# pygda-team/pygda

Hardware: AMD Instinct MI355X
Metric: edges_aggregated_per_sec (higher is better)
Workload: dtype f32

## Files before the change

include/gda_hip.h:

```cpp
#ifndef GDA_HIP_H
#define GDA_HIP_H

#include <stddef.h>
#include <stdint.h>

#ifdef __cplusplus
extern "C" {
#endif

#define GDA_OK 0
#define GDA_E_NULL (-1)
#define GDA_E_SIZE (-2)
#define GDA_E_WORKSPACE (-3)
#define GDA_E_UNSUPPORTED (-4)
#define GDA_E_ALIAS (-5)
#define GDA_E_RCCL (-100)

typedef void* gda_stream_t;

int gda_abi_version(void);
const char* gda_status_string(int status);

size_t gda_graph_workspace_bytes(int64_t E, int64_t N);
int gda_build_csr_norm(const int64_t* src, const int64_t* dst, const float* w,
// ... 430 lines not shown
                             const int32_t* idx_s, const int32_t* idx_t, const float* alpha, int64_t n_i,
                             int a, float dropout_p, uint64_t seed, const int64_t* step, uint32_t site,
                             float gp_weight, float* loss, const gda_adam_tensor* params ,
                             float lr, float beta1, float beta2, float eps, float weight_decay,
                             void* workspace, size_t workspace_bytes, gda_stream_t stream);

#define GDA_GEMM_NT 0
#define GDA_GEMM_NN 1
#define GDA_GEMM_TN 2
size_t gda_gemm_workspace_bytes(int mode, int64_t M, int64_t N, int64_t K);
int gda_gemm_f32(int mode, int64_t M, int64_t N, int64_t K, const float* A, int64_t lda,
                 const float* B, int64_t ldb, float* C, int64_t ldc,
                 void* workspace, size_t workspace_bytes, gda_stream_t stream);
int gda_gemm_ex_f32(int mode, int64_t M, int64_t N, int64_t K, const float* A, int64_t lda,
                    const float* B, int64_t ldb, float* C, int64_t ldc, const float* bias, float* colsum,
                    void* workspace, size_t workspace_bytes, gda_stream_t stream);
size_t gda_gemm_tall_workspace_bytes(int mode, int64_t M, int64_t N, int64_t K);
size_t gda_gemm_skinny_workspace_bytes(int mode, int64_t M, int64_t N, int64_t K);
int gda_gemm_skinny_f32(int mode, int64_t M, int64_t N, int64_t K, const float* A, int64_t lda,
                        const float* B, int64_t ldb, float* C, int64_t ldc, const float* bias, float* colsum,
                        void* workspace, size_t workspace_bytes, gda_stream_t stream);
int gda_gemm_nn_mask_f32(int64_t M, int64_t N, int64_t K, const float* A, int64_t lda, const float* B, int64_t ldb,
                         float* C, int64_t ldc, const float* y, int64_t ldm, float p, gda_stream_t stream);
int gda_gemm_tall_fwd_ex_f32(int64_t M, int64_t N, int64_t K, const float* A, int64_t lda, const int64_t* arow,
                             const float* B, int64_t ldb, float* C, int64_t ldc, const float* bias,
                             int act_mode, float p, uint64_t seed, const int64_t* step_dev, uint32_t site0,
                             uint32_t site1, gda_stream_t stream);
int gda_gemm_tall_wgrad_gather_f32(int64_t N, int64_t Krows, const float* A, int64_t lda, const float* X, int64_t ldx,
                                   const int64_t* xrow, float* C, int64_t ldc, float* colsum,
                                   void* workspace, size_t workspace_bytes, gda_stream_t stream);
int gda_gemm_tall_f32(int mode, int64_t M, int64_t N, int64_t K, const float* A, int64_t lda,
                      const float* B, int64_t ldb, float* C, int64_t ldc, const float* bias, float* colsum,
                      void* workspace, size_t workspace_bytes, gda_stream_t stream);


size_t gda_softmax_nll_workspace_bytes(void);
int gda_softmax_entropy_fwd_f32(const float* logits, int64_t ld, int64_t N, int C, float clamp_min, float* loss,
                                void* workspace, size_t workspace_bytes, gda_stream_t stream);
int gda_softmax_entropy_bwd_f32(const float* logits, int64_t ld, int64_t N, int C, float clamp_min,
                                const float* grad_loss, float* grad_logits, int64_t ldg, gda_stream_t stream);
int gda_softmax_nll_fwd_f32(const float* logits, int64_t ld, const int64_t* labels, int64_t N, int C,
                            float* loss, void* workspace, size_t workspace_bytes, gda_stream_t stream);
int gda_softmax_nll_fwd_ex_f32(const float* logits, int64_t ld, const int64_t* labels, int64_t N, int C,
                               float* loss, double* stats, void* workspace, size_t workspace_bytes,
                               gda_stream_t stream);
int gda_softmax_nll_bwd_f32(const float* logits, int64_t ld, const int64_t* labels, int64_t N, int C,
// ... 148 lines not shown
```

pygda_amd/_lib.py:

```python
import ctypes
import os
from ctypes import c_char_p, c_float, c_int, c_int64, c_size_t, c_void_p

import torch

HERE = os.path.dirname(os.path.abspath(__file__))
LIB_PATH = os.path.join(HERE, "libgda_hip.so")

class _P(c_void_p):

    @classmethod
    def from_param(cls, obj):
        if isinstance(obj, torch.Tensor):
            return c_void_p(obj.data_ptr())
        if obj is None:
            return None
        if isinstance(obj, str):
            raise TypeError("a str is not a pointer argument")
        return c_void_p.from_param(obj)


_SIGNATURES = {
    "gda_abi_version": (c_int, []),
    "gda_status_string": (c_char_p, [c_int]),
# ... 89 lines not shown
                                   _P, _P, _P, c_float, _P, _P, _P, c_int64, _P, _P, _P, c_int64, _P,
                                   _P, c_size_t, _P]),
    "gda_mmd_fused_nseg": (c_int, [c_int, c_int64, c_int64, c_float, c_int]),
    "gda_mmd_fused_layout": (c_int, [c_int, c_int64, c_int64, _P, c_int]),
    "gda_mmd_fused_fwd_f32": (c_int, [_P, c_int64, _P, c_int64, c_int64, _P, _P, c_int, c_int64, c_float, c_int, c_float,
                                      c_float, _P, _P, _P, _P, _P, _P, c_int, _P, c_size_t, _P]),
    "gda_mmd_fused_bwd_f32": (c_int, [_P, c_int, c_int, c_int64, c_int64, _P, c_float, _P,
                                      _P, _P, c_int64, _P, _P, _P, c_int64, _P, _P]),
    "gda_mmd_fused_bwd_mask_f32": (c_int, [_P, c_int, c_int, c_int64, c_int64, _P, c_float, _P,
                                           _P, _P, c_int64, _P, _P, _P, c_int64, _P, _P, c_float, _P, c_float, _P]),
    "gda_copy_from_pinned": (c_int, [_P, _P, c_size_t, _P]),
    "gda_softmax_entropy_fwd_f32": (c_int, [_P, c_int64, c_int64, c_int, c_float, _P, _P, c_size_t, _P]),
    "gda_softmax_entropy_bwd_f32": (c_int, [_P, c_int64, c_int64, c_int, c_float, _P, _P, c_int64, _P]),
    "gda_mmd_chunked_plan": (c_int, [c_int, c_int64, c_int64, c_float, c_int, _P, c_int]),
    "gda_mmd_chunked_workspace_bytes": (c_size_t, [c_int, c_int64, c_int64]),
    "gda_mmd_chunked_fwd_f32": (c_int, [_P, c_int64, _P, c_int64, c_int64, _P, _P, c_int, c_int64, c_float, c_int, c_float,
                                        c_float, _P, _P, _P, c_int64, _P, _P, _P, c_int64, c_int, _P, c_size_t, _P]),
    "gda_mmd_fused_bwd_ld_f32": (c_int, [_P, c_int64, c_int, c_int, c_int64, c_int64, _P, c_float, _P,
                                         _P, _P, c_int64, _P, _P, _P, c_int64, _P, _P, c_float, _P, c_float, _P]),
    "gda_gemm_tall_fwd_ex_f32": (c_int, [c_int64, c_int64, c_int64, _P, c_int64, _P, _P, c_int64, _P, c_int64, _P, c_int,
                                         c_float, ctypes.c_uint64, _P, ctypes.c_uint32, ctypes.c_uint32, _P]),
    "gda_gemm_tall_wgrad_gather_f32": (c_int, [c_int64, c_int64, _P, c_int64, _P, c_int64, _P, _P, c_int64, _P, _P, c_size_t, _P]),
    "gda_gemm_nn_mask_f32": (c_int, [c_int64, c_int64, c_int64, _P, c_int64, _P, c_int64, _P, c_int64, _P, c_int64, c_float, _P]),
    "gda_grl_disc_workspace_bytes": (c_size_t, [c_int64, c_int64, c_int]),
    "gda_grl_mlp_ce_workspace_bytes": (c_size_t, [c_int64, c_int64]),
    "gda_lsgan_head_workspace_bytes": (c_size_t, [c_int64]),
    "gda_lsgan_head_fwd_f32": (c_int, [_P, c_int64, c_int64, c_int64, _P, _P, c_float, _P, _P, _P, c_size_t, _P]),
    "gda_lsgan_head_bwd_f32": (c_int, [_P, c_int64, c_int64, c_int64, _P, _P, c_float, _P, _P, c_int64, _P, _P,
                                       _P, c_size_t, _P]),
    "gda_grl_mlp_ce_fwd_f32": (c_int, [_P, c_int64, c_int64, _P, c_int64, c_int64, c_int64, c_int64, _P, _P, _P, _P,
                                       c_float, ctypes.c_uint64, _P, ctypes.c_uint32, _P, _P, c_size_t, _P]),
    "gda_grl_mlp_ce_bwd_f32": (c_int, [_P, c_int64, c_int64, _P, c_int64, c_int64, c_int64, c_int64, _P, _P, _P, _P,
                                       c_float, ctypes.c_uint64, _P, ctypes.c_uint32, _P, c_int, c_float, _P,
                                       _P, _P, _P, _P, _P, _P, _P, c_size_t, _P]),
    "gda_mlp_head_fwd_f32": (c_int, [c_int, _P, c_int64, c_int64, _P, c_int64, c_int64, c_int64, c_int64, _P, _P, _P, _P,
                                     c_float, ctypes.c_uint64, _P, ctypes.c_uint32, _P, _P, c_size_t, _P]),
    "gda_mlp_head_bwd_f32": (c_int, [c_int, _P, c_int64, c_int64, _P, c_int64, c_int64, c_int64, c_int64, _P, _P, _P, _P,
                                     c_float, ctypes.c_uint64, _P, ctypes.c_uint32, _P, c_int, c_float, _P,
                                     _P, _P, _P, _P, _P, _P, _P, c_size_t, _P]),
    "gda_grl_disc_ce_fwd_f32": (c_int, [_P, c_int64, c_int64, _P, c_int64, c_int64, c_int64, c_int,
                                        _P, _P, _P, _P, _P, _P, c_size_t, _P]),
    "gda_grl_disc_ce_bwd_f32": (c_int, [_P, c_int64, c_int64, _P, c_int64, c_int64, c_int64, c_int,
                                        _P, _P, _P, _P, c_float, _P, _P, _P, _P, _P, c_size_t, _P]),
    "gda_relu_dropout_fwd_f32": (c_int, [_P, _P, c_int64, c_float, ctypes.c_uint64, _P, ctypes.c_uint32, _P]),
    "gda_relu_dropout_bwd_f32": (c_int, [_P, _P, _P, c_int64, c_float, _P]),
    "gda_relu_dropout_tiled_fwd_f32": (c_int, [_P, c_int64, c_int64, _P, c_float, ctypes.c_uint64, _P, ctypes.c_uint32, _P]),
# ... 237 lines not shown
```

pygda_amd/csrc/gda_gemm.hip:

```cpp
#include "gda_common.h"
#include "gda_dropout.h"

#include <cstdlib>

namespace {

constexpr int TB = 256;
constexpr int TILE = 64;
constexpr int DK = 32;
constexpr int LDT = TILE + 4;
constexpr int PF = 4;

using f32x16 = __attribute__((ext_vector_type(16))) float;

__device__ __forceinline__ float4 ld4(const float* __restrict__ p, int64_t ld, int64_t r, int64_t c,
                                      int64_t rows, int64_t cols, bool vec) {
    float4 v = make_float4(0.f, 0.f, 0.f, 0.f);
    if (r >= rows) return v;
    const float* q = p + r * ld + c;
    if (vec && c + 3 < cols) return *reinterpret_cast<const float4*>(q);
    if (c + 0 < cols) v.x = q[0];
    if (c + 1 < cols) v.y = q[1];
    if (c + 2 < cols) v.z = q[2];
    if (c + 3 < cols) v.w = q[3];
// ... 508 lines not shown
        float c = 0.f;
#pragma unroll
        for (int q = 0; q < SK_N; ++q) if (q == n) { a = acc[q]; c = cs[q]; }
        *reinterpret_cast<float4*>(red + 4 * threadIdx.x) = a;
        __syncthreads();
        if (rl == 0) {
            float4 t = make_float4(0.f, 0.f, 0.f, 0.f);
            for (int r = 0; r < rlanes; ++r) {
                const float4 u = *reinterpret_cast<const float4*>(red + 4 * (r * pieces + p));
                t.x += u.x; t.y += u.y; t.z += u.z; t.w += u.w;
            }
            *reinterpret_cast<float4*>(out + (int64_t)n * K + 4 * p) = t;
        }
        if (CS) {
            __syncthreads();
            if (p == 0) red[rl] = c;
            __syncthreads();
            if (threadIdx.x == 0) {
                float t = 0.f;
                for (int r = 0; r < rlanes; ++r) t += red[r];
                CS[(int64_t)blockIdx.x * N + n] = t;
            }
        }
    }
}

bool vec_ok(const float* p, int64_t ld) { return ld % 4 == 0 && ((uintptr_t)p & 15) == 0; }

int slabs_for(int64_t K) {
    const int per = 128, cap = 256;
    int64_t s = gda_cdiv(K, per);
    if (s < 1) s = 1;
    if (s > cap) s = cap;
    return (int)s;
}

}

bool split_k(int mode, int64_t M, int64_t N, int64_t K) {
    return mode == GDA_GEMM_TN || (mode == GDA_GEMM_NN && K >= 1024 && M <= 512 && N <= 512);
}

extern "C" size_t gda_gemm_workspace_bytes(int mode, int64_t M, int64_t N, int64_t K) {
    if (M <= 0 || N <= 0 || K <= 0 || !split_k(mode, M, N, K)) return 0;
    const int s = slabs_for(K);
    return s > 1 ? (size_t)s * (size_t)M * (size_t)(N + 1) * sizeof(float) : 0;
// ... 197 lines not shown
        k_skinny_fwd<<<(unsigned)blocks, TB, 0, stream>>>(A, lda, B, ldb, bias, C, ldc, M, (int)N, (int)K);
    } else if (mode == GDA_GEMM_NN) {
        if (K > SK_N || !wide_ok(N) || bias || colsum || !al(B, ldb) || !al(C, ldc) || lda < K || ldb < N) return GDA_E_UNSUPPORTED;
        const int64_t rpb = TB / (N / 4);
        const int64_t blocks = min(gda_cdiv(M, rpb), (int64_t)256 * 16);
        k_skinny_dgrad<<<(unsigned)blocks, TB, 0, stream>>>(A, lda, B, ldb, C, ldc, M, (int)K, (int)N);
    } else if (mode == GDA_GEMM_TN) {
        if (M > SK_N || !wide_ok(N) || bias || !al(B, ldb) || lda < M || ldb < N) return GDA_E_UNSUPPORTED;
        const int64_t slabs = skinny_slabs(K);
        const int64_t rows = gda_cdiv(K, slabs);
        if (!workspace || workspace_bytes < gda_gemm_skinny_workspace_bytes(mode, M, N, K)) return GDA_E_WORKSPACE;
        float* part = (float*)workspace;
        float* cs_part = part + (size_t)slabs * M * N;
        k_skinny_wgrad<<<(unsigned)slabs, TB, 0, stream>>>(A, lda, B, ldb, part, colsum ? cs_part : nullptr, K, rows, (int)M, (int)N);
        GDA_LAUNCH_CHECK();
        GDA_UNLESS_SKIPPED("k_slab_sum") k_slab_sum<<<(unsigned)gda_cdiv(M * N + (colsum ? M : 0), SS_OUT), TB, 0, stream>>>(part, (int)slabs, M, N, C, ldc, cs_part, colsum);
    } else {
        return GDA_E_UNSUPPORTED;
    }
    GDA_LAUNCH_CHECK();
    return GDA_OK;
}

extern "C" int gda_gemm_nn_mask_f32(int64_t M, int64_t N, int64_t K, const float* A, int64_t lda, const float* B, int64_t ldb,
                                    float* C, int64_t ldc, const float* y, int64_t ldm, float p, gda_stream_t stream_) {
    if (M <= 0 || N <= 0 || K <= 0 || ldc < N || ldm < N || lda < K || ldb < N) return GDA_E_SIZE;
    if (!A || !B || !C || !y) return GDA_E_NULL;
    if (C == A || C == B || C == y) return GDA_E_ALIAS;
    if (!(p >= 0.f && p < 1.f)) return GDA_E_SIZE;
    if (ldc % 4 || ldm % 4 || ldb % 4 || (((uintptr_t)C | (uintptr_t)y | (uintptr_t)B) & 15)) return GDA_E_UNSUPPORTED;
    hipStream_t stream = (hipStream_t)stream_;
    const float mscale = 1.f / (1.f - p);
    if (K <= SK_N && (N == 32 || N == 64 || N == 128 || N == 256)) {
        const int64_t rpb = TB / (N / 4);
        const int64_t blocks = min(gda_cdiv(M, rpb), (int64_t)256 * 16);
        k_skinny_dgrad<<<(unsigned)blocks, TB, 0, stream>>>(A, lda, B, ldb, C, ldc, M, (int)K, (int)N, y, ldm, mscale);
        GDA_LAUNCH_CHECK();
        return GDA_OK;
    }
    static const bool split16 = [] { const char* e = std::getenv("PYGDA_AMD_GEMM_SPLIT_F16"); return !(e && e[0] == '0'); }();
    if (!split16 || (N != 128 && N != 256) || (K != 128 && K != 256) || lda % 4 || ((uintptr_t)A & 15)) return GDA_E_UNSUPPORTED;
    const int64_t bm = K == 128 ? 128 : 64;
    const int64_t nt = gda_cdiv(M, bm);
    const dim3 g((unsigned)min(nt, (int64_t)256), (unsigned)(N / 128));
    const size_t img = (size_t)bm * (K + 8) * 2;
    const size_t lds = 4 * img + 2 * (size_t)bm * sizeof(float);
// ... 61 lines not shown
```

pygda_amd/models/a2gnn.py:

```python
import numpy as np
import torch
import torch.nn.functional as F

from ..nn import A2GNNBase
from ..ops import grl_disc_ce, source_ce
from ..utils import MMD
from .base import BaseGDA


import contextlib

_null = contextlib.nullcontext


EARLY_CE_BACKWARD = True


class A2GNN(BaseGDA):
    def __init__(self, in_dim, hid_dim, num_classes, mode='node', num_layers=3, dropout=0.,
                 act=F.relu, s_pnums=0, t_pnums=30, adv=False, weight=5, weight_decay=0., lr=4e-3,
                 epoch=200, device='cuda:0', batch_size=0, num_neigh=-1, verbose=2, **kwargs):
        super().__init__(in_dim=in_dim, hid_dim=hid_dim, num_classes=num_classes, num_layers=num_layers,
                         dropout=dropout, act=act, weight_decay=weight_decay, lr=lr, epoch=epoch,
                         device=device, batch_size=batch_size, num_neigh=num_neigh, verbose=verbose,
                         **kwargs)
        self.s_pnums, self.t_pnums, self.adv, self.weight, self.mode = s_pnums, t_pnums, adv, weight, mode
        self.compute_target_logits = True
        self.overlap_streams = True
        self.overlap_sampled = True
        self._auto_reorder_ok = type(self) is A2GNN

    def init_model(self, **kwargs):
        return A2GNNBase(in_dim=self.in_dim, hid_dim=self.hid_dim, num_classes=self.num_classes,
                         num_layers=self.num_layers, adv=self.adv, dropout=self.dropout, act=self.act,
                         mode=self.mode, **kwargs).to(self.device)

    def _target_logits_async(self, net, target_data, h0, after):
        main = torch.cuda.current_stream()
        side = getattr(self, "_side_stream", None)
        if side is None:
            side = self._side_stream = torch.cuda.Stream()
        side.wait_event(after)
        with torch.cuda.stream(side), torch.no_grad():
            feats = net.feat_bottleneck_from(h0.detach(), target_data.edge_index, None, self.t_pnums, draw=1)
            out = net.feat_classifier(feats, target_data.edge_index, None, 1)
        out.record_stream(main)
        return out, side

    def _source_branch(self, source_data):
        net = self.a2gnn
        sb = None if self.mode == 'node' else source_data.batch
        h0_s = net.first_conv(source_data.x, source_data.edge_index, self.s_pnums,
                              draws="stacked" if (self.s_pnums <= 0 and getattr(source_data, "n_id", None) is not None) else 0)
        source_features, feats = net.feat_pair_from(h0_s, source_data.edge_index, sb, self.s_pnums)
        source_logits = net.feat_classifier(feats, source_data.edge_index, sb, 1)
        loss = self._gmean(source_ce(source_logits, source_data.y), source_logits.size(0))
        from .. import hipgraph
        self._early = self._src_ready = None
        if (EARLY_CE_BACKWARD and hipgraph.defer_total and type(self) is A2GNN and not self.adv and self.mode == 'node'
                and torch.is_grad_enabled() and feats.requires_grad):
            cls_params = [p for p in net.cls.parameters() if p.requires_grad]
            self._src_ready = torch.cuda.Event()
            self._src_ready.record()
            grads = torch.autograd.grad(loss, [feats] + cls_params)
            self._early = (feats, grads[0], cls_params, grads[1:])
            loss = loss.detach()
        return loss, source_logits, source_features
# ... 149 lines not shown
```

pygda_amd/nn/a2gnn_base.py:

```python
import torch.nn.functional as F
from torch import nn

from .prop_gcn_conv import PropGCNConv
from .reverse_layer import GradReverse
from .linear import DenseLinear


def global_mean_pool(x, batch, size=None):
    from ..ops import segment_mean
    if size is None:
        size = getattr(batch, "_gda_num_graphs", None)
    return segment_mean(x, batch, size)


class ActPair:
    __slots__ = ("draws",)

    def __init__(self, a, b=None):
        self.draws = (a, b)

    def detach(self):
        return ActPair(self.draws[0].detach(), None if self.draws[1] is None else self.draws[1].detach())


# ... 51 lines not shown
        conv = self.convs[0]
        if draws == "stacked":
            hit = conv.forward_stacked(x, self.dropout, self.training, 2) \
                if (prop_nums <= 0 and self.act is F.relu and self.mode == "node" and self.hid_dim % 4 == 0) else None
            if hit is not None:
                return StackedAct(hit)
            draws = 0
        if draws and self.act is F.relu and self.mode == "node" and prop_nums > 0:
            hit = conv.forward_act(x, edge_index, prop_nums, self.dropout, self.training, pair=draws > 1)
            if hit is not None:
                return ActPair(*hit) if draws > 1 else ActPair(hit)
        return conv.forward_colmajor(x, edge_index, prop_nums) if self._fused_act(x) else conv(x, edge_index, prop_nums)

    def _fused_act(self, x):
        return self.act is F.relu and x.is_cuda and self.mode == "node"

    def _act_dropout(self, x):
        from ..ops import ColMajor
        if isinstance(x, ColMajor) or (self.act is F.relu and x.is_cuda):
            from ..ops import relu_dropout
            return relu_dropout(x, self.dropout, self.training)
        return F.dropout(self.act(x), p=self.dropout, training=self.training)

    def feat_bottleneck_from(self, h0, edge_index, batch, prop_nums=30, draw=0):
        if isinstance(h0, ActPair):
            x = h0.draws[draw] if h0.draws[draw] is not None else h0.draws[0]
        else:
            x = self._act_dropout(h0)
        for conv in self.convs[1:]:
            hit = conv.forward_act(x, edge_index, prop_nums, self.dropout, self.training) \
                if (self.act is F.relu and self.mode == "node" and prop_nums > 0) else None
            if hit is not None:
                x = hit
                continue
            x = self._act_dropout(conv.forward_colmajor(x, edge_index, prop_nums) if self._fused_act(x)
                                  else conv(x, edge_index, prop_nums))
        if self.mode == "graph":
            x = global_mean_pool(x, batch)
        return x

    def feat_pair_from(self, h0, edge_index, batch, prop_nums=30):
        from ..ops import relu_dropout_pair, relu_dropout_pair_ok, split_halves
        stacked = isinstance(h0, StackedAct)
        if not stacked and not (prop_nums <= 0 and self.mode == "node" and self.act is F.relu and relu_dropout_pair_ok(h0)
                                and self.hid_dim % 4 == 0):
            return (self.feat_bottleneck_from(h0, edge_index, batch, prop_nums),
                    self.feat_bottleneck_from(h0, edge_index, batch, prop_nums))
        x = h0.y if stacked else relu_dropout_pair(h0, self.dropout, self.training)
        rest = list(self.convs[1:])
        for conv in rest[:-1]:
            hit = conv.forward_stacked(x, self.dropout, self.training, 1) if stacked else None
            x = hit if hit is not None else self._act_dropout(conv(x, edge_index, prop_nums))
        if rest:
            from ..ops import relu_dropout_split
            hit = rest[-1].forward_stacked(x, self.dropout, self.training, 3) if stacked else None
            if hit is not None:
                return hit
            return relu_dropout_split(rest[-1](x, edge_index, prop_nums), self.dropout, self.training)
        return split_halves(x)

    def feat_classifier(self, x, edge_index, batch, prop_nums=1):
        return self.cls(x, edge_index, prop_nums) if self.mode == "node" else self.cls(x)

    def domain_classifier(self, x, alpha):
        return self.domain_discriminator(GradReverse.apply(x, alpha))
```

pygda_amd/nn/linear.py:

```python
import math

import torch
import torch.nn.functional as F
from torch import nn

from .. import sparse_features


def glorot(t):
    if t is not None:
        a = math.sqrt(6.0 / (t.size(-2) + t.size(-1)))
        with torch.no_grad():
            t.uniform_(-a, a)


def zeros(t):
    if t is not None:
        with torch.no_grad():
            t.fill_(0)


class _TallLinear(torch.autograd.Function):

    @staticmethod
    def forward(ctx, x, weight):
        from ..ops import GEMM_NT, gemm, sink_of
        ctx.sink = sink_of(x)
        ctx.save_for_backward(x, weight)
        return gemm(GEMM_NT, x, weight)

    @staticmethod
    def backward(ctx, gy):
        from ..ops import GEMM_NN, GEMM_TN, gemm, masked_dgrad
        x, weight = ctx.saved_tensors
        gy = gy.contiguous()
        gx = None
        if ctx.needs_input_grad[0]:
            gx = masked_dgrad(gy, weight, ctx.sink) if ctx.sink is not None else gemm(GEMM_NN, gy, weight)
        gw = gemm(GEMM_TN, gy, x) if ctx.needs_input_grad[1] else None
        return gx, gw


# ... 69 lines not shown
        self.bias = nn.Parameter(torch.empty(out_channels)) if bias else None
        self.reset_parameters()

    def reset_parameters(self):
        if self.weight_initializer == "glorot":
            glorot(self.weight)
        else:
            bound = math.sqrt(6 / ((1 + math.sqrt(5) ** 2) * self.in_channels))
            with torch.no_grad():
                self.weight.uniform_(-bound, bound)
        if self.bias is not None:
            if self.weight_initializer == "glorot":
                zeros(self.bias)
            else:
                b = 1.0 / math.sqrt(self.in_channels)
                with torch.no_grad():
                    self.bias.uniform_(-b, b)

    def tall_gemm_ok(self, x):
        if self.bias is not None or x.dim() != 2 or not x.is_cuda or x.dtype != torch.float32:
            return False
        if x.size(1) >= sparse_features.MIN_WIDTH and sparse_features.lookup(x) is not None:
            return False
        return 1024 <= x.size(0) and self.in_channels <= 256 and self.out_channels <= 256

    def forward(self, x):
        if self.bias is None and x.dim() == 2 and x.size(1) >= sparse_features.MIN_WIDTH:
            sf = sparse_features.lookup(x)
            if sf is not None:
                return sparse_features.sparse_linear(self.weight, sf)
        if (self.bias is None and x.dim() == 2 and x.is_cuda and x.dtype == torch.float32 and x.size(0) >= 1024
                and self.in_channels <= 256 and self.out_channels <= 256):
            return _TallLinear.apply(x, self.weight)
        if x.is_cuda and x.dtype == torch.float32 and self.weight.dtype == torch.float32 and x.dim() >= 1:
            rows = x.reshape(-1, x.size(-1))
            y = _TallLinear.apply(rows, self.weight) if self.bias is None else _TallLinearBias.apply(rows, self.weight, self.bias)
            return y if x.dim() == 2 else y.view(*x.shape[:-1], self.out_channels)
        return F.linear(x, self.weight, self.bias)

    def __repr__(self):
        return f"{self.__class__.__name__}({self.in_channels}, {self.out_channels}, bias={self.bias is not None})"
```

pygda_amd/nn/prop_gcn_conv.py:

```python
import torch
from torch import nn

from .. import sparse_features
from ..graph import CSRGraph, as_graph, build_csr
from ..ops import propagate
from .linear import Linear, zeros

SPARSE_COLMAJOR = True


def gcn_norm(edge_index, edge_weight=None, num_nodes=None, improved=False, add_self_loops=True,
             dtype=None):
    if num_nodes is None:
        num_nodes = int(edge_index.max()) + 1 if edge_index.numel() else 0
    g = build_csr(edge_index, num_nodes, edge_weight, improved, add_self_loops, True, "col")
    return g.to_coo()


class PropGCNConv(nn.Module):
    def __init__(self, in_channels, out_channels, improved=False, cached=False,
                 add_self_loops=True, normalize=True, bias=True, **kwargs):
        super().__init__()
        self.in_channels, self.out_channels = in_channels, out_channels
        self.improved, self.cached = improved, cached
# ... 34 lines not shown
            return None
        return tall_linear_act(x, self.lin.weight, self.bias, p, training, mode)

    def forward_act(self, x, edge_index, prop_nums, p, training, pair=False):
        from ..ops import GatheredRows, propagate_act, propagate_act_ok, tall_fused_ok, tall_linear_act
        gathered = isinstance(x, GatheredRows)
        if prop_nums <= 0 or not (isinstance(x, torch.Tensor) or gathered) or not x.is_cuda or x.dim() != 2:
            return None
        g = self._graph(x, edge_index, None)
        if getattr(g, "n_interior", None) is None or getattr(g, "iplan", None) is None or self.out_channels % 4:
            return None
        if gathered:
            out = tall_linear_act(x, self.lin.weight, None, 0.0, False, 0) if tall_fused_ok(x, self.lin.weight) \
                else self.lin(x.dense())
        else:
            out = self.lin(x)
        if not propagate_act_ok(out, g, prop_nums, self.bias):
            from ..ops import relu_dropout
            pre = propagate(out, g, prop_nums, self.bias)
            a = relu_dropout(pre, p, training)
            return (a, relu_dropout(pre.detach(), p, training)) if pair else a
        return propagate_act(out, g, prop_nums, self.bias, p, training, pair)

    def _forward(self, x, edge_index, prop_nums, edge_weight, colmajor_out):
        from ..ops import GatheredRows
        if isinstance(x, GatheredRows):
            x = x.dense()
        if colmajor_out and prop_nums > 0 and self.lin.tall_gemm_ok(x):
            from ..ops import lds_kstep_plan, tall_linear_colmajor
            g = self._graph(x, edge_index, edge_weight)
            if (self.out_channels % 4 == 0 and lds_kstep_plan(g, prop_nums, False) is not None
                    and lds_kstep_plan(g, prop_nums, True) is not None):
                return propagate(tall_linear_colmajor(x, self.lin.weight), g, prop_nums, self.bias)
        if (colmajor_out and prop_nums > 0 and x.dim() == 2 and x.size(1) >= sparse_features.MIN_WIDTH
                and self.out_channels % 4 == 0 and SPARSE_COLMAJOR):
            sf = sparse_features.lookup(x)
            if sf is not None:
                from ..ops import lds_kstep_plan
                g = self._graph(x, edge_index, edge_weight)
                if lds_kstep_plan(g, prop_nums, False) is not None and lds_kstep_plan(g, prop_nums, True) is not None:
                    hT = sparse_features.sparse_linear_colmajor(self.lin.weight, sf)
                    if hT is not None:
                        return propagate(hT, g, prop_nums, self.bias)
        if prop_nums <= 0 and self.bias is not None and self.lin.tall_gemm_ok(x):
            from .linear import tall_linear_bias
            return tall_linear_bias(x, self.lin.weight, self.bias)
# ... 15 lines not shown
```

pygda_amd/ops.py:

```python
import ctypes
import weakref

import os as _os

import torch

from . import _lib, profiler
from .graph import CSRGraph, build_csr


def _f32c(t, name):
    _lib.require_gpu_tensor(t, name)
    if t.dtype != torch.float32:
        raise _lib.GdaError(f"{name}: the aggregation path computes in fp32, got {t.dtype}")
    return t.contiguous()


GRAD_SINKS = True
_sinks_on = False
sink_hits = 0


class grad_sinks:

# ... 406 lines not shown
def lds_kstep_plan(graph, K, transposed=False):
    from .graph import KSTEP_LDS, KSTEP_LDS_MIN_K
    if not KSTEP_LDS or K < KSTEP_LDS_MIN_K or not graph.static:
        return None
    return graph.kstep_plan(transposed)


class _TallLinearT(torch.autograd.Function):

    @staticmethod
    def forward(ctx, x, weight):
        x, weight = _f32c(x, "x"), _f32c(weight, "weight")
        n, k = x.shape
        out = weight.size(0)
        n_pad = (n + 3) // 4 * 4
        hT = torch.empty(out, n_pad, dtype=torch.float32, device=x.device)
        gemm_raw(GEMM_NT, out, n, k, weight, k, x, k, hT, n_pad, f"dense_projection[{k}x{out}]")
        ctx.save_for_backward(x, weight)
        return hT

    @staticmethod
    def backward(ctx, gT):
        x, weight = ctx.saved_tensors
        n, k = x.shape
        out = weight.size(0)
        gT = gT.contiguous()
        n_pad = gT.size(1)
        gx = gw = None
        if ctx.needs_input_grad[0]:
            gx = torch.empty(n, k, dtype=torch.float32, device=x.device)
            gemm_raw(GEMM_TN, n, k, out, gT, n_pad, weight, k, gx, k, f"dense_projection_dgrad[{out}x{k}]")
        if ctx.needs_input_grad[1]:
            gw = torch.empty(out, k, dtype=torch.float32, device=x.device)
            gemm_raw(GEMM_NN, out, k, n, gT, n_pad, x, k, gw, k, f"dense_projection_wgrad[{out}x{k}]")
        return gx, gw


def tall_linear_colmajor(x, weight):
    return ColMajor(_TallLinearT.apply(x, weight), x.size(0))


_colsum_hint = None


def colsum(x):
    global _colsum_hint
    hint, _colsum_hint = _colsum_hint, None
    if hint is not None and hint[0] == x.data_ptr() and hint[2].shape == x.shape and x.is_contiguous():
        return hint[1]
    if not (x.is_cuda and x.dtype == torch.float32 and x.dim() == 2 and 0 < x.size(1) <= 1024 and x.stride(1) == 1):
        return x.sum(0)
    n, d = x.shape
    out = torch.empty(d, dtype=torch.float32, device=x.device)
    ws, nbytes = _lib.scratch("gda_colsum_workspace_bytes", x.device, "colsum", n, d)
    _lib.call("gda_colsum_f32", x, x.stride(0), n, d, out, ws, nbytes, _lib.stream())
    return out


class _PropagateT(torch.autograd.Function):

    @staticmethod
    def forward(ctx, x, bias, graph, K, x_colmajor=False):
# ... 826 lines not shown
        if ctx.sink is not None and ctx.sink.mine(gy):
            return gy, None
        gy = gy.contiguous()
        gx = torch.empty_like(gy)
        _lib.call("gda_relu_dropout_bwd_f32", gy, y, gx, gy.numel(), ctx.p, _lib.stream())
        return gx, None


class _ReluDropoutT(torch.autograd.Function):

    @staticmethod
    def forward(ctx, xT, n, p):
        d, n_pad = xT.shape
        y = torch.empty(n, d, dtype=torch.float32, device=xT.device)
        _lib.call("gda_relu_dropout_fwd_cm_f32", xT, n_pad, y, n, d, float(p), *dropout_state.generator(xT.device),
                  _lib.stream())
        ctx.save_for_backward(y)
        ctx.p, ctx.n_pad = float(p), n_pad
        return y

    @staticmethod
    def backward(ctx, gy):
        (y,) = ctx.saved_tensors
        n, d = y.shape
        gy = gy.contiguous()
        gxT = torch.empty(d, ctx.n_pad, dtype=torch.float32, device=gy.device)
        if ctx.n_pad != n:
            gxT[:, n:].zero_()
        _lib.call("gda_relu_dropout_bwd_cm_f32", gy, y, gxT, ctx.n_pad, n, d, ctx.p, _lib.stream())
        return gxT, None, None


class _ReluDropoutPair(torch.autograd.Function):

    @staticmethod
    def forward(ctx, x, p):
        x = _f32c(x, "x")
        n, d = x.shape
        y = torch.empty(2 * n, d, dtype=torch.float32, device=x.device)
        _lib.call("gda_relu_dropout_pair_fwd_f32", x, y, n, d, float(p), *dropout_state.generator(x.device, sites=2),
                  _lib.stream())
        ctx.save_for_backward(y)
        ctx.p = float(p)
        return y

    @staticmethod
    def backward(ctx, gy):
        (y,) = ctx.saved_tensors
        n, d = y.size(0) // 2, y.size(1)
        gy = gy.contiguous()
        gx = torch.empty(n, d, dtype=torch.float32, device=gy.device)
        cs = ws = None
        nbytes = 0
# ... 2262 lines not shown
```

Before: 3.335 billion.

## Fuse ReLU-dropout activation into consumer GEMMs for column-major preactivations

Adds two HIP kernels that apply ReLU and dropout to column-major preactivations while loading them as GEMM operands. One is an MFMA tall GEMM that can also write the activated output for backward; the other is a skinny classifier GEMM. The A2GNN bottleneck and classifier paths now pass raw preactivations to the next layer instead of running a separate activation kernel, which removes one full read and write of the hidden matrix per layer. The cost is more complex routing with fallbacks, and the per-element dropout RNG inside the GEMM must match the standalone kernel's masks.

Result: faster. 3.439 billion, median of 6 (+3.1%).

```diff
diff --git a/include/gda_hip.h b/include/gda_hip.h
--- a/include/gda_hip.h
+++ b/include/gda_hip.h
@@ -476,6 +476,12 @@
                         void* workspace, size_t workspace_bytes, gda_stream_t stream);
 int gda_gemm_nn_mask_f32(int64_t M, int64_t N, int64_t K, const float* A, int64_t lda, const float* B, int64_t ldb,
                          float* C, int64_t ldc, const float* y, int64_t ldm, float p, gda_stream_t stream);
+int gda_gemm_act_cm_f32(int64_t n, int64_t M, int64_t K, const float* xT, int64_t ldT, const float* W, int64_t ldw,
+                        float* y, float* hT, int64_t ldc, float p, uint64_t seed, const int64_t* step, uint32_t site,
+                        gda_stream_t stream);
+int gda_gemm_skinny_act_cm_f32(int64_t n, int64_t N, int64_t K, const float* xT, int64_t ldT, const float* W, int64_t ldw,
+                               float* Y, int64_t ldy, float p, uint64_t seed, const int64_t* step, uint32_t site,
+                               gda_stream_t stream);
 int gda_gemm_tall_fwd_ex_f32(int64_t M, int64_t N, int64_t K, const float* A, int64_t lda, const int64_t* arow,
                              const float* B, int64_t ldb, float* C, int64_t ldc, const float* bias,
                              int act_mode, float p, uint64_t seed, const int64_t* step_dev, uint32_t site0,
diff --git a/pygda_amd/_lib.py b/pygda_amd/_lib.py
--- a/pygda_amd/_lib.py
+++ b/pygda_amd/_lib.py
@@ -135,6 +135,10 @@
                                          c_float, ctypes.c_uint64, _P, ctypes.c_uint32, ctypes.c_uint32, _P]),
     "gda_gemm_tall_wgrad_gather_f32": (c_int, [c_int64, c_int64, _P, c_int64, _P, c_int64, _P, _P, c_int64, _P, _P, c_size_t, _P]),
     "gda_gemm_nn_mask_f32": (c_int, [c_int64, c_int64, c_int64, _P, c_int64, _P, c_int64, _P, c_int64, _P, c_int64, c_float, _P]),
+    "gda_gemm_act_cm_f32": (c_int, [c_int64, c_int64, c_int64, _P, c_int64, _P, c_int64, _P, _P, c_int64, c_float,
+                                    ctypes.c_uint64, _P, ctypes.c_uint32, _P]),
+    "gda_gemm_skinny_act_cm_f32": (c_int, [c_int64, c_int64, c_int64, _P, c_int64, _P, c_int64, _P, c_int64, c_float,
+                                           ctypes.c_uint64, _P, ctypes.c_uint32, _P]),
     "gda_grl_disc_workspace_bytes": (c_size_t, [c_int64, c_int64, c_int]),
     "gda_grl_mlp_ce_workspace_bytes": (c_size_t, [c_int64, c_int64]),
     "gda_lsgan_head_workspace_bytes": (c_size_t, [c_int64]),
diff --git a/pygda_amd/csrc/gda_gemm.hip b/pygda_amd/csrc/gda_gemm.hip
--- a/pygda_amd/csrc/gda_gemm.hip
+++ b/pygda_amd/csrc/gda_gemm.hip
@@ -554,6 +554,150 @@
                 CS[(int64_t)blockIdx.x * N + n] = t;
             }
         }
+    }
+}
+
+constexpr int AC_BM = 128;
+constexpr int AC_BN = 32;
+constexpr int AC_LDW = AC_BM + 4, AC_LDX = AC_BN + 4;
+
+__global__ void __launch_bounds__(TB)
+k_gemm_act_cm(const float* __restrict__ xT, int64_t ldT, const float* __restrict__ W, int64_t ldw, float* __restrict__ y,
+              float* __restrict__ hT, int64_t ldc, int64_t n, int64_t M, int64_t K, float p, float scale, uint64_t seed,
+              const int64_t* __restrict__ step, uint32_t site) {
+    __shared__ __attribute__((aligned(16))) float Ws[DK][AC_LDW];
+    __shared__ __attribute__((aligned(16))) float Xs[DK][AC_LDX];
+    const int tid = threadIdx.x, wave = tid >> 6, lane = tid & 63;
+    const int ka = lane >> 5, la = lane & 31;
+    const int64_t i0 = (int64_t)blockIdx.x * AC_BN;
+    const bool drop = p > 0.f;
+    const uint64_t st = drop ? (uint64_t)step[0] : 0;
+    const uint32_t thresh = dropout_thresh(p);
+    const int wr = tid >> 3, wk = (tid & 7) * 4;
+    const int xi = tid & 31, xq = tid >> 5;
+    const int64_t node = i0 + xi;
+    const bool node_in = node < n;
+    const float* xcol = xT + (node_in ? node : n - 1);
+    const int yr = tid >> 3, yc = (tid & 7) * 4;
+    for (int64_t m0 = 0; m0 < M; m0 += AC_BM) {
+        f32x16 acc;
+#pragma unroll
+        for (int r = 0; r < 16; ++r) acc[r] = 0.f;
+        const bool store_y = y != nullptr && m0 == 0;
+        float4 vw[PF][4];
+        float vx[PF][4];
+#define AC_LOAD(C_, K0_)                                                                                   \
+    {                                                                                                      \
+        _Pragma("unroll") for (int q = 0; q < 4; ++q)                                                      \
+            vw[C_][q] = ld4_fast(W, ldw, m0 + wr + 32 * q, (K0_) + wk, M, K);                              \
+        const int64_t kx = (K0_) + 4 * xq;                                                                 \
+        const bool in = node_in && kx < K;                    \
+        const int64_t kc = kx < K ? kx : K - 4;                                                            \
+        _Pragma("unroll") for (int e = 0; e < 4; ++e) {                                                    \
+            const float v = xcol[(kc + e) * ldT];                                                          \
+            vx[C_][e] = in ? v : 0.f;                                                                      \
+        }                                                                                                  \
+    }
+#pragma unroll
+        for (int c = 0; c < PF; ++c)
+            if ((int64_t)c * DK < K) AC_LOAD(c, (int64_t)c * DK)
+        for (int64_t kb = 0; kb < K; kb += PF * DK) {
+#pragma unroll
+            for (int c = 0; c < PF; ++c) {
+                const int64_t k0 = kb + c * DK;
+                if (k0 >= K) break;
+                __syncthreads();
+#pragma unroll
+                for (int q = 0; q < 4; ++q) {
+                    const int r = wr + 32 * q;
+                    Ws[wk + 0][r] = vw[c][q].x; Ws[wk + 1][r] = vw[c][q].y; Ws[wk + 2][r] = vw[c][q].z; Ws[wk + 3][r] = vw[c][q].w;
+                }
+                {
+                    const float4 v = make_float4(vx[c][0], vx[c][1], vx[c][2], vx[c][3]);
+                    float4 o;
+                    if (drop) {
+                        uint32_t rn[4];
+                        dropout_draw(seed, st, site, (uint64_t)((node * K + k0 + 4 * xq) >> 2), rn);
+                        o = relu_keep(v, rn, thresh, scale);
+                    } else {
+                        o = make_float4(v.x > 0.f ? v.x : 0.f, v.y > 0.f ? v.y : 0.f, v.z > 0.f ? v.z : 0.f, v.w > 0.f ? v.w : 0.f);
+                    }
+                    Xs[4 * xq + 0][xi] = o.x; Xs[4 * xq + 1][xi] = o.y; Xs[4 * xq + 2][xi] = o.z; Xs[4 * xq + 3][xi] = o.w;
+                }
+                if (k0 + PF * DK < K) AC_LOAD(c, k0 + PF * DK)
+                __syncthreads();
+                if (store_y && i0 + yr < n && k0 + yc < K)
+                    *reinterpret_cast<float4*>(y + (i0 + yr) * K + k0 + yc) =
+                        make_float4(Xs[yc + 0][yr], Xs[yc + 1][yr], Xs[yc + 2][yr], Xs[yc + 3][yr]);
+#pragma unroll
+                for (int kk = 0; kk < DK; kk += 2)
+                    acc = __builtin_amdgcn_mfma_f32_32x32x2f32(Ws[kk + ka][32 * wave + la], Xs[kk + ka][la], acc, 0, 0, 0);
+            }
+        }
+#undef AC_LOAD
+        const int64_t j = i0 + la;
+#pragma unroll
+        for (int r = 0; r < 16; ++r) {
+            const int64_t m = m0 + 32 * wave + (r & 3) + 8 * (r >> 2) + 4 * ka;
+            if (m < M && j < n) hT[m * ldc + j] = acc[r];
+        }
+    }
+}
+
+constexpr int SA_NODES = 64, SA_TB = 8 * SA_NODES;
+
+template <int PIECES >
+__global__ void __launch_bounds__(SA_TB)
+k_skinny_fwd_act_cm(const float* __restrict__ xT, int64_t ldT, const float* __restrict__ W, int64_t ldw, float* __restrict__ Y,
+                    int64_t ldy, int64_t n, int N, float p, float scale, uint64_t seed, const int64_t* __restrict__ step,
+                    uint32_t site) {
+    constexpr int K = 32 * PIECES;
+    __shared__ __attribute__((aligned(16))) float Ws[SK_N * K];
+    __shared__ float part[8][SA_NODES * (SK_N + 1)];
+    for (int i = threadIdx.x; i < N * K; i += SA_TB) Ws[i] = W[(int64_t)(i / K) * ldw + i % K];
+    const int j = threadIdx.x >> 6, lane = threadIdx.x & 63;
+    const int64_t node = (int64_t)blockIdx.x * SA_NODES + lane;
+    const float* xcol = xT + (node < n ? node : n - 1);
+    const bool drop = p > 0.f;
+    const uint64_t st = drop ? (uint64_t)step[0] : 0;
+    const uint32_t thresh = dropout_thresh(p);
+    float v[PIECES][4];
+#pragma unroll
+    for (int t = 0; t < PIECES; ++t)
+#pragma unroll
+        for (int e = 0; e < 4; ++e) v[t][e] = xcol[(int64_t)(4 * (j + 8 * t) + e) * ldT];
+    __syncthreads();
+    float acc[SK_N];
+#pragma unroll
+    for (int c = 0; c < SK_N; ++c) acc[c] = 0.f;
+#pragma unroll
+    for (int t = 0; t < PIECES; ++t) {
+        const int pc = j + 8 * t;
+        float4 a = make_float4(v[t][0], v[t][1], v[t][2], v[t][3]);
+        if (drop) {
+            uint32_t rn[4];
+            dropout_draw(seed, st, site, (uint64_t)((node * K + 4 * pc) >> 2), rn);
+            a = relu_keep(a, rn, thresh, scale);
+        } else {
+            a = make_float4(a.x > 0.f ? a.x : 0.f, a.y > 0.f ? a.y : 0.f, a.z > 0.f ? a.z : 0.f, a.w > 0.f ? a.w : 0.f);
+        }
+#pragma unroll
+        for (int c = 0; c < SK_N; ++c)
+            if (c < N) {
+                const float4 w = *reinterpret_cast<const float4*>(Ws + c * K + 4 * pc);
+                acc[c] = fmaf(a.x, w.x, acc[c]); acc[c] = fmaf(a.y, w.y, acc[c]);
+                acc[c] = fmaf(a.z, w.z, acc[c]); acc[c] = fmaf(a.w, w.w, acc[c]);
+            }
+    }
+#pragma unroll
+    for (int c = 0; c < SK_N; ++c) part[j][lane * (SK_N + 1) + c] = acc[c];
+    __syncthreads();
+    const int ln = threadIdx.x >> 3, c = threadIdx.x & 7;
+    const int64_t row = (int64_t)blockIdx.x * SA_NODES + ln;
+    if (c < N && row < n) {
+        const int o = ln * (SK_N + 1) + c;
+        Y[row * ldy + c] = ((part[0][o] + part[1][o]) + (part[2][o] + part[3][o])) +
+                           ((part[4][o] + part[5][o]) + (part[6][o] + part[7][o]));
     }
 }
 
@@ -797,6 +941,43 @@
     return GDA_OK;
 }
 
+extern "C" int gda_gemm_act_cm_f32(int64_t n, int64_t M, int64_t K, const float* xT, int64_t ldT, const float* W, int64_t ldw,
+                                   float* y, float* hT, int64_t ldc, float p, uint64_t seed, const int64_t* step,
+                                   uint32_t site, gda_stream_t stream_) {
+    if (n < 0 || M < 0 || K < 0 || ldT < n || ldc < n || ldw < K || !(p >= 0.f && p < 1.f)) return GDA_E_SIZE;
+    if (n == 0 || M == 0) return GDA_OK;
+    if (!xT || !W || !hT || !step) return GDA_E_NULL;
+    if (hT == xT || hT == W || (y && (y == xT || y == W || y == hT))) return GDA_E_ALIAS;
+    if (K < 4 || K % 4 || M % 4 || ldw % 4 || (((uintptr_t)W | (uintptr_t)y) & 15)) return GDA_E_UNSUPPORTED;
+    const int64_t blocks = gda_cdiv(n, AC_BN);
+    if (blocks > INT32_MAX) return GDA_E_SIZE;
+    GDA_UNLESS_SKIPPED("k_gemm_act_cm") k_gemm_act_cm<<<(unsigned)blocks, TB, 0, (hipStream_t)stream_>>>(
+        xT, ldT, W, ldw, y, hT, ldc, n, M, K, p, 1.f / (1.f - p), seed, step, site);
+    GDA_LAUNCH_CHECK();
+    return GDA_OK;
+}
+
+extern "C" int gda_gemm_skinny_act_cm_f32(int64_t n, int64_t N, int64_t K, const float* xT, int64_t ldT, const float* W,
+                                          int64_t ldw, float* Y, int64_t ldy, float p, uint64_t seed, const int64_t* step,
+                                          uint32_t site, gda_stream_t stream_) {
+    if (n < 0 || N < 0 || K < 0 || ldT < n || ldy < N || ldw < K || !(p >= 0.f && p < 1.f)) return GDA_E_SIZE;
+    if (n == 0 || N == 0) return GDA_OK;
+    if (!xT || !W || !Y || !step) return GDA_E_NULL;
+    if (Y == xT || Y == W) return GDA_E_ALIAS;
+    if (N > SK_N || (K != 32 && K != 64 && K != 128 && K != 256)) return GDA_E_UNSUPPORTED;
+    const int64_t blocks = gda_cdiv(n, SA_NODES);
+    if (blocks > INT32_MAX) return GDA_E_SIZE;
+    hipStream_t stream = (hipStream_t)stream_;
+    const float scale = 1.f / (1.f - p);
+#define SA_LAUNCH(P_) k_skinny_fwd_act_cm<P_><<<(unsigned)blocks, SA_TB, 0, stream>>>(xT, ldT, W, ldw, Y, ldy, n, (int)N, p, scale, seed, step, site)
+    GDA_UNLESS_SKIPPED("k_skinny_fwd_act_cm") {
+        if (K == 32) SA_LAUNCH(1); else if (K == 64) SA_LAUNCH(2); else if (K == 128) SA_LAUNCH(4); else SA_LAUNCH(8);
+    }
+#undef SA_LAUNCH
+    GDA_LAUNCH_CHECK();
+    return GDA_OK;
+}
+
 extern "C" int gda_gemm_nn_mask_f32(int64_t M, int64_t N, int64_t K, const float* A, int64_t lda, const float* B, int64_t ldb,
                                     float* C, int64_t ldc, const float* y, int64_t ldm, float p, gda_stream_t stream_) {
     if (M <= 0 || N <= 0 || K <= 0 || ldc < N || ldm < N || lda < K || ldb < N) return GDA_E_SIZE;
diff --git a/pygda_amd/models/a2gnn.py b/pygda_amd/models/a2gnn.py
--- a/pygda_amd/models/a2gnn.py
+++ b/pygda_amd/models/a2gnn.py
@@ -42,7 +42,8 @@
             side = self._side_stream = torch.cuda.Stream()
         side.wait_event(after)
         with torch.cuda.stream(side), torch.no_grad():
-            feats = net.feat_bottleneck_from(h0.detach(), target_data.edge_index, None, self.t_pnums, draw=1)
+            feats = net.feat_bottleneck_from(h0.detach(), target_data.edge_index, None, self.t_pnums, draw=1,
+                                             preact_out=True)
             out = net.feat_classifier(feats, target_data.edge_index, None, 1)
         out.record_stream(main)
         return out, side
diff --git a/pygda_amd/nn/a2gnn_base.py b/pygda_amd/nn/a2gnn_base.py
--- a/pygda_amd/nn/a2gnn_base.py
+++ b/pygda_amd/nn/a2gnn_base.py
@@ -97,19 +97,31 @@
             return relu_dropout(x, self.dropout, self.training)
         return F.dropout(self.act(x), p=self.dropout, training=self.training)
 
-    def feat_bottleneck_from(self, h0, edge_index, batch, prop_nums=30, draw=0):
+    def feat_bottleneck_from(self, h0, edge_index, batch, prop_nums=30, draw=0, preact_out=False):
+        from ..ops import ColMajor
+        pre = x = None
         if isinstance(h0, ActPair):
             x = h0.draws[draw] if h0.draws[draw] is not None else h0.draws[0]
         else:
-            x = self._act_dropout(h0)
+            pre = h0
         for conv in self.convs[1:]:
+            if pre is not None:
+                nxt = conv.forward_from_preact(pre, edge_index, prop_nums, self.dropout, self.training) \
+                    if (isinstance(pre, ColMajor) and self.act is F.relu and self.mode == "node") else None
+                if nxt is not None:
+                    pre = nxt
+                    continue
+                x, pre = self._act_dropout(pre), None
             hit = conv.forward_act(x, edge_index, prop_nums, self.dropout, self.training) \
                 if (self.act is F.relu and self.mode == "node" and prop_nums > 0) else None
             if hit is not None:
                 x = hit
                 continue
-            x = self._act_dropout(conv.forward_colmajor(x, edge_index, prop_nums) if self._fused_act(x)
-                                  else conv(x, edge_index, prop_nums))
+            pre = conv.forward_colmajor(x, edge_index, prop_nums) if self._fused_act(x) else conv(x, edge_index, prop_nums)
+        if pre is not None:
+            if preact_out and isinstance(pre, ColMajor) and self.mode == "node":
+                return pre
+            x = self._act_dropout(pre)
         if self.mode == "graph":
             x = global_mean_pool(x, batch)
         return x
@@ -135,6 +147,13 @@
         return split_halves(x)
 
     def feat_classifier(self, x, edge_index, batch, prop_nums=1):
+        from ..ops import ColMajor
+        if isinstance(x, ColMajor):
+            hit = self.cls.forward_logits_from_preact(x, edge_index, prop_nums, self.dropout, self.training) \
+                if self.mode == "node" else None
+            if hit is not None:
+                return hit
+            x = self._act_dropout(x)
         return self.cls(x, edge_index, prop_nums) if self.mode == "node" else self.cls(x)
 
     def domain_classifier(self, x, alpha):
diff --git a/pygda_amd/nn/linear.py b/pygda_amd/nn/linear.py
--- a/pygda_amd/nn/linear.py
+++ b/pygda_amd/nn/linear.py
@@ -18,6 +18,9 @@
     if t is not None:
         with torch.no_grad():
             t.fill_(0)
+
+
+TALL_MIN_ROWS = 1024
 
 
 class _TallLinear(torch.autograd.Function):
@@ -133,7 +136,7 @@
             return False
         if x.size(1) >= sparse_features.MIN_WIDTH and sparse_features.lookup(x) is not None:
             return False
-        return 1024 <= x.size(0) and self.in_channels <= 256 and self.out_channels <= 256
+        return TALL_MIN_ROWS <= x.size(0) and self.in_channels <= 256 and self.out_channels <= 256
 
     def forward(self, x):
         if self.bias is None and x.dim() == 2 and x.size(1) >= sparse_features.MIN_WIDTH:
diff --git a/pygda_amd/nn/prop_gcn_conv.py b/pygda_amd/nn/prop_gcn_conv.py
--- a/pygda_amd/nn/prop_gcn_conv.py
+++ b/pygda_amd/nn/prop_gcn_conv.py
@@ -80,6 +80,27 @@
             return (a, relu_dropout(pre.detach(), p, training)) if pair else a
         return propagate_act(out, g, prop_nums, self.bias, p, training, pair)
 
+    def forward_from_preact(self, pre, edge_index, prop_nums, p, training):
+        from .. import ops
+        from . import linear
+        lin = self.lin
+        if not (prop_nums > 0 and lin.bias is None and pre.size(0) >= linear.TALL_MIN_ROWS and lin.in_channels <= 256
+                and lin.out_channels <= 256 and self.out_channels % 4 == 0 and ops.act_tall_linear_ok(pre, lin.weight)):
+            return None
+        g = self._graph(pre, edge_index, None)
+        if getattr(g, "n_interior", None) is not None and getattr(g, "iplan", None) is not None:
+            return None
+        if ops.lds_kstep_plan(g, prop_nums, False) is None or ops.lds_kstep_plan(g, prop_nums, True) is None:
+            return None
+        return propagate(ops.act_tall_linear_colmajor(pre, lin.weight, p, training), g, prop_nums, self.bias)
+
+    def forward_logits_from_preact(self, pre, edge_index, prop_nums, p, training):
+        from .. import ops
+        if prop_nums <= 0 or self.lin.bias is not None or not ops.act_skinny_ok(pre, self.lin.weight):
+            return None
+        out = ops.act_skinny_linear(pre, self.lin.weight, p, training)
+        return propagate(out, self._graph(pre, edge_index, None), prop_nums, self.bias)
+
     def _forward(self, x, edge_index, prop_nums, edge_weight, colmajor_out):
         from ..ops import GatheredRows
         if isinstance(x, GatheredRows):
diff --git a/pygda_amd/ops.py b/pygda_amd/ops.py
--- a/pygda_amd/ops.py
+++ b/pygda_amd/ops.py
@@ -452,22 +452,85 @@
     @staticmethod
     def backward(ctx, gT):
         x, weight = ctx.saved_tensors
-        n, k = x.shape
-        out = weight.size(0)
-        gT = gT.contiguous()
-        n_pad = gT.size(1)
-        gx = gw = None
-        if ctx.needs_input_grad[0]:
-            gx = torch.empty(n, k, dtype=torch.float32, device=x.device)
-            gemm_raw(GEMM_TN, n, k, out, gT, n_pad, weight, k, gx, k, f"dense_projection_dgrad[{out}x{k}]")
-        if ctx.needs_input_grad[1]:
-            gw = torch.empty(out, k, dtype=torch.float32, device=x.device)
-            gemm_raw(GEMM_NN, out, k, n, gT, n_pad, x, k, gw, k, f"dense_projection_wgrad[{out}x{k}]")
-        return gx, gw
+        return _tall_linear_t_backward(x, weight, gT, ctx.needs_input_grad[0], ctx.needs_input_grad[1])
+
+
+def _tall_linear_t_backward(x, weight, gT, want_x, want_w):
+    n, k = x.shape
+    out = weight.size(0)
+    gT = gT.contiguous()
+    n_pad = gT.size(1)
+    gx = gw = None
+    if want_x:
+        gx = torch.empty(n, k, dtype=torch.float32, device=x.device)
+        gemm_raw(GEMM_TN, n, k, out, gT, n_pad, weight, k, gx, k, f"dense_projection_dgrad[{out}x{k}]")
+    if want_w:
+        gw = torch.empty(out, k, dtype=torch.float32, device=x.device)
+        gemm_raw(GEMM_NN, out, k, n, gT, n_pad, x, k, gw, k, f"dense_projection_wgrad[{out}x{k}]")
+    return gx, gw
 
 
 def tall_linear_colmajor(x, weight):
     return ColMajor(_TallLinearT.apply(x, weight), x.size(0))
+
+
+ACT_IN_CONSUMER = True
+
+
+class _ActTallLinearT(torch.autograd.Function):
+
+    @staticmethod
+    def forward(ctx, xT, n, weight, p, keep):
+        weight = _f32c(weight, "weight")
+        k, n_pad = xT.shape
+        out = weight.size(0)
+        y = torch.empty(n, k, dtype=torch.float32, device=xT.device) if keep else None
+        hT = torch.empty(out, n_pad, dtype=torch.float32, device=xT.device)
+        with profiler.region(f"dense_projection[{k}x{out}]", 1, 4 * (k * n + out * k + out * n + (n * k if keep else 0)),
+                             2 * out * n * k):
+            _lib.call("gda_gemm_act_cm_f32", n, out, k, xT, n_pad, weight, k, y, hT, n_pad, float(p),
+                      *dropout_state.generator(xT.device), _lib.stream())
+        if keep:
+            ctx.save_for_backward(y, weight)
+        ctx.p, ctx.n_pad = float(p), n_pad
+        return hT
+
+    @staticmethod
+    def backward(ctx, gT):
+        y, weight = ctx.saved_tensors
+        gy, gw = _tall_linear_t_backward(y, weight, gT, ctx.needs_input_grad[0], ctx.needs_input_grad[2])
+        gxT = _relu_dropout_t_backward(y, gy, ctx.p, ctx.n_pad) if gy is not None else None
+        return gxT, None, gw, None, None
+
+
+def act_tall_linear_ok(x, weight):
+    return (ACT_IN_CONSUMER and isinstance(x, ColMajor) and x.t.is_cuda and x.t.dtype == torch.float32
+            and x.t.is_contiguous() and weight.dtype == torch.float32 and weight.dim() == 2 and weight.is_contiguous()
+            and weight.size(1) == x.size(1) and x.n >= 1 and weight.size(1) % 4 == 0 and weight.size(1) >= 4
+            and weight.size(0) % 4 == 0 and weight.data_ptr() % 16 == 0)
+
+
+def act_tall_linear_colmajor(x, weight, p, training):
+    keep = torch.is_grad_enabled() and (x.t.requires_grad or weight.requires_grad)
+    return ColMajor(_ActTallLinearT.apply(x.t, x.n, weight, float(p) if training else 0.0, keep), x.n)
+
+
+def act_skinny_ok(x, weight):
+    return (ACT_IN_CONSUMER and isinstance(x, ColMajor) and x.t.is_cuda and x.t.dtype == torch.float32
+            and x.t.is_contiguous() and not (torch.is_grad_enabled() and (x.t.requires_grad or weight.requires_grad))
+            and weight.dtype == torch.float32 and weight.dim() == 2 and weight.is_contiguous()
+            and weight.size(1) == x.size(1) and x.n >= SKINNY_ROWS and weight.size(0) <= 8
+            and weight.size(1) in (32, 64, 128, 256))
+
+
+def act_skinny_linear(x, weight, p, training):
+    n, k = x.shape
+    c = weight.size(0)
+    out = torch.empty(n, c, dtype=torch.float32, device=x.t.device)
+    with profiler.region(f"dense_projection[{k}x{c}]", 1, 4 * (k * n + c * k + n * c), 2 * n * c * k):
+        _lib.call("gda_gemm_skinny_act_cm_f32", n, c, k, x.t, x.t.size(1), weight.detach(), k, out, c,
+                  float(p) if training else 0.0, *dropout_state.generator(x.t.device), _lib.stream())
+    return out
 
 
 _colsum_hint = None
@@ -1340,13 +1403,17 @@
     @staticmethod
     def backward(ctx, gy):
         (y,) = ctx.saved_tensors
-        n, d = y.shape
-        gy = gy.contiguous()
-        gxT = torch.empty(d, ctx.n_pad, dtype=torch.float32, device=gy.device)
-        if ctx.n_pad != n:
-            gxT[:, n:].zero_()
-        _lib.call("gda_relu_dropout_bwd_cm_f32", gy, y, gxT, ctx.n_pad, n, d, ctx.p, _lib.stream())
-        return gxT, None, None
+        return _relu_dropout_t_backward(y, gy, ctx.p, ctx.n_pad), None, None
+
+
+def _relu_dropout_t_backward(y, gy, p, n_pad):
+    n, d = y.shape
+    gy = gy.contiguous()
+    gxT = torch.empty(d, n_pad, dtype=torch.float32, device=gy.device)
+    if n_pad != n:
+        gxT[:, n:].zero_()
+    _lib.call("gda_relu_dropout_bwd_cm_f32", gy, y, gxT, n_pad, n, d, p, _lib.stream())
+    return gxT
 
 
 class _ReluDropoutPair(torch.autograd.Function):
```
